# colmap/glomap

Hardware: NVIDIA H100
Metric: observations/sec per BA LM-iteration (higher is better)
Workload: dtype f64

## Files before the change

glomap_b200/csrc/ba_kernels.cuh:

```cuda
#pragma once
#include "common.cuh"
#include "pcg.cuh"

namespace b200 {

constexpr int kCamRec = 8;
constexpr int kIntrRec = 8;
constexpr double kZEps = 1e-12;
constexpr int kSeg = 256;
__host__ __device__ constexpr int seg_split(int n) { return n <= 0 ? 0 : (n < kSeg + kSeg / 2 ? 1 : (n + kSeg / 2) / kSeg); }
constexpr int kIntrSmem = 16;
constexpr int kJpDoubles = 6;
constexpr int kSensorRec = 16;

struct BAView {
  int C, P, K;
  long long N;
  int n_tiles;
  int n_segs;
  int min_views;
  const int* obs_cam;
  const int* obs_pt;
  const double2* obs_xy;
  const unsigned* pt_begin;
// ... 35 lines not shown
  }
}

struct Intr {
  double fx, fy, cx, cy, k1, k2;
  int model;
};
__device__ __forceinline__ Intr ld_intr(const double* __restrict__ ir) {
  return Intr{ir[0], ir[1], ir[2], ir[3], ir[4], ir[5], (int)ir[6]};
}

struct ProjJac {
  double iz, u, v, m00, m01, m10, m11;
};

__device__ __forceinline__ void project_jac(const Intr& in, double x, double y, double z, double& px, double& py,
                                            ProjJac& pj) {
  const double iz = 1.0 / z;
  const double u = x * iz, v = y * iz;
  pj.iz = iz;
  pj.u = u;
  pj.v = v;
  if (in.k1 == 0.0 && in.k2 == 0.0) {
    px = in.fx * u + in.cx;
    py = in.fy * v + in.cy;
    pj.m00 = in.fx; pj.m01 = 0.0; pj.m10 = 0.0; pj.m11 = in.fy;
  } else {
    const double r2 = u * u + v * v;
    const double d = 1.0 + r2 * (in.k1 + in.k2 * r2);
    const double dd = in.k1 + 2.0 * in.k2 * r2;
    px = in.fx * u * d + in.cx;
    py = in.fy * v * d + in.cy;
    const double a00 = d + 2.0 * u * u * dd, a01 = 2.0 * u * v * dd, a11 = d + 2.0 * v * v * dd;
    pj.m00 = in.fx * a00; pj.m01 = in.fx * a01; pj.m10 = in.fy * a01; pj.m11 = in.fy * a11;
  }
}
__device__ __forceinline__ void project_only(const Intr& in, double x, double y, double z, double& px, double& py) {
  const double iz = 1.0 / z;
  const double u = x * iz, v = y * iz;
  if (in.k1 == 0.0 && in.k2 == 0.0) {
    px = in.fx * u + in.cx;
    py = in.fy * v + in.cy;
  } else {
    const double r2 = u * u + v * v;
    const double d = 1.0 + r2 * (in.k1 + in.k2 * r2);
    px = in.fx * u * d + in.cx;
    py = in.fy * v * d + in.cy;
  }
}
// ... 91 lines not shown
  for (int a = 0; a < 2; ++a) {
    const double j0 = J[3 * a], j1 = J[3 * a + 1], j2 = J[3 * a + 2];
    o.Jr[3 * a + 0] = rvar ? -2.0 * (j1 * rz - j2 * ry) : 0.0;
    o.Jr[3 * a + 1] = rvar ? -2.0 * (j2 * rx - j0 * rz) : 0.0;
    o.Jr[3 * a + 2] = rvar ? -2.0 * (j0 * ry - j1 * rx) : 0.0;
  }
#pragma unroll
  for (int a = 0; a < 2; ++a)
#pragma unroll
    for (int b = 0; b < 3; ++b) o.Jp[3 * a + b] = J[3 * a] * R[b] + J[3 * a + 1] * R[3 + b] + J[3 * a + 2] * R[6 + b];
}

struct ObsCore {
  double J[6], e[2], rho0, rho1, RX[3], R[9];
  double uv[2];
  ProjJac pj;
  bool valid;
};
__device__ __forceinline__ void obs_core_R(const double R[9], const double4& t4, const Intr& in,
                                           const double* __restrict__ sr, double X0, double X1, double X2, double2 xy,
                                           double huber_a, ObsCore& o) {
#pragma unroll
  for (int k = 0; k < 9; ++k) o.R[k] = R[k];
  o.RX[0] = o.R[0] * X0 + o.R[1] * X1 + o.R[2] * X2;
  o.RX[1] = o.R[3] * X0 + o.R[4] * X1 + o.R[5] * X2;
  o.RX[2] = o.R[6] * X0 + o.R[7] * X1 + o.R[8] * X2;
  double xc = o.RX[0] + t4.x, yc = o.RX[1] + t4.y, zc = o.RX[2] + t4.z;
  if (sr) sensor_apply(sr, xc, yc, zc);
  o.valid = zc > kZEps;
  if (!o.valid) {
#pragma unroll
    for (int k = 0; k < 6; ++k) o.J[k] = 0.0;
    o.e[0] = o.e[1] = 0.0;
    o.rho0 = 0.0;
    o.rho1 = 0.0;
    o.uv[0] = o.uv[1] = 0.0;
    o.pj = ProjJac{0.0, 0.0, 0.0, 0.0, 0.0, 0.0, 0.0};
    return;
  }
  double px, py;
  project_jac(in, xc, yc, zc, px, py, o.pj);
  proj_jac_rows(o.pj, o.J);
  o.uv[0] = xc / zc;
  o.uv[1] = yc / zc;
  if (sr) {
#pragma unroll
    for (int a = 0; a < 2; ++a) {
      const double j0 = o.J[3 * a], j1 = o.J[3 * a + 1], j2 = o.J[3 * a + 2];
      o.J[3 * a] = j0 * sr[0] + j1 * sr[3] + j2 * sr[6];
      o.J[3 * a + 1] = j0 * sr[1] + j1 * sr[4] + j2 * sr[7];
      o.J[3 * a + 2] = j0 * sr[2] + j1 * sr[5] + j2 * sr[8];
    }
  }
  o.e[0] = px - xy.x;
// ... 755 lines not shown
```

glomap_b200/csrc/ba_kernels_v2.cuh:

```cuda
#pragma once
#include "ba_kernels.cuh"
#include "pcg.cuh"

namespace b200 {

struct BAViewV2 {
  const double* Ap;
  double* z4;
  const double* pts4;
  double* Ufk = nullptr;
  const IntrVarRec* ivar = nullptr;
  int C = 0;
};

template <int NK>
__device__ __forceinline__ void obs_intr_jac(const ObsCore& o, const Intr& in, const IntrVarRec& iv,
                                             double Jk[2][NK > 0 ? NK : 1]) {
#pragma unroll
  for (int j = 0; j < NK; ++j) {
    double jx = 0.0, jy = 0.0;
    if (j < iv.mb) intr_param_jac(in, iv.pidx[j], o.uv[0], o.uv[1], 1.0, jx, jy);
    if (!o.valid) jx = jy = 0.0;
    Jk[0][j] = jx;
    Jk[1][j] = jy;
  }
}
template <int NK>
__device__ __forceinline__ void obs_intr_rows(const ObsCore& o, const Intr& in, const IntrVarRec& iv,
                                              const double Jp[6], double Jk[2][NK > 0 ? NK : 1],
                                              double B[NK > 0 ? 3 * NK : 1]) {
  obs_intr_jac<NK>(o, in, iv, Jk);
#pragma unroll
  for (int j = 0; j < NK; ++j)
#pragma unroll
    for (int c = 0; c < 3; ++c) B[3 * j + c] = o.rho1 * (Jp[c] * Jk[0][j] + Jp[3 + c] * Jk[1][j]);
}

struct SegRec {
  double R[9];
  double4 t4;
  Intr in;
  const double* sr;
};
__device__ __forceinline__ void seg_records(const BAView& v, int seg, int cam, const double* __restrict__ cam_rec,
                                            const double* __restrict__ intr_rec, SegRec& s) {
  const double4 q4 = ld_rec32(cam_rec + (size_t)cam * kCamRec);
  s.t4 = ld_rec32(cam_rec + (size_t)cam * kCamRec + 4);
  s.in = ld_intr(intr_rec + (size_t)v.seg_intr[seg] * kIntrRec);
  s.sr = sensor_of_seg(v, seg);
  const double q[4] = {q4.x, q4.y, q4.z, q4.w};
  quat_to_R(q, s.R);
}
__device__ __forceinline__ void to_sensor(const double* __restrict__ sr, double x[3]) {
  if (!sr) return;
  const double x0 = x[0], x1 = x[1], x2 = x[2];
#pragma unroll
  for (int k = 0; k < 3; ++k) x[k] = sr[3 * k] * x0 + sr[3 * k + 1] * x1 + sr[3 * k + 2] * x2;
}
__device__ __forceinline__ void cam_frame_jac(const ObsCore& o, const double r[3], double a[2], double w[3]) {
  const ProjJac& p = o.pj;
  const double t0 = r[0] - p.u * r[2], t1 = r[1] - p.v * r[2];
  const double c = o.rho1 * p.iz;
  a[0] = c * (p.m00 * t0 + p.m01 * t1);
  a[1] = c * (p.m10 * t0 + p.m11 * t1);
  const double s0 = p.iz * (p.m00 * a[0] + p.m10 * a[1]), s1 = p.iz * (p.m01 * a[0] + p.m11 * a[1]);
  w[0] = s0;
  w[1] = s1;
  w[2] = -(p.u * s0 + p.v * s1);
}
__device__ __forceinline__ void rig_to_frame(const double* __restrict__ sr, double x[3]) {
  const double x0 = x[0], x1 = x[1], x2 = x[2];
#pragma unroll
  for (int k = 0; k < 3; ++k) x[k] = sr[k] * x0 + sr[3 + k] * x1 + sr[6 + k] * x2;
}

constexpr int kXqStride = 8;
__global__ void ba2_pack_x(int C, const double* __restrict__ x, const double* __restrict__ cam_rec,
                           double* __restrict__ xp) {
  const int c = blockIdx.x * blockDim.x + threadIdx.x;
  if (c >= C) return;
  const double* r = cam_rec + (size_t)c * kCamRec;
  const double q[4] = {r[0], r[1], r[2], r[3]};
  double R[9];
// ... 68 lines not shown
  const bool tvar = !(cmask & 2), rvar = !(cmask & 1);
  constexpr int NKK = NK > 0 ? NK : 1;
  const int blk = v.seg_intr[warp];
  IntrVarRec iv{};
  if (NK > 0) iv = v2.ivar[blk];
  double Ukk[NKK * (NKK + 1) / 2], gk[NKK], Ufk[6][NKK];
#pragma unroll
  for (int k = 0; k < NKK * (NKK + 1) / 2; ++k) Ukk[k] = 0.0;
#pragma unroll
  for (int k = 0; k < NKK; ++k) {
    gk[k] = 0.0;
#pragma unroll
    for (int i2 = 0; i2 < 6; ++i2) Ufk[i2][k] = 0.0;
  }
  const double* __restrict__ pts4 = v2.pts4;
  int i = b + lane;
  int pt_nxt = 0;
  double2 xy = make_double2(0, 0);
  double4 Xc = make_double4(0, 0, 0, 0);
  if (i < e) {
    const int pt0 = ld_stream(v.pt_c + i);
    if (i + 32 < e) pt_nxt = ld_stream(v.pt_c + i + 32);
    xy = ld_stream(v.xy_c + i);
    Xc = ld_rec32(pts4 + 4 * (size_t)pt0);
  }
  for (; i < e; i += 32) {
    double4 Xn = Xc;
    double2 xyn = xy;
    int pt_nn = 0;
    if (i + 32 < e) {
      Xn = ld_rec32(pts4 + 4 * (size_t)pt_nxt);
      xyn = ld_stream(v.xy_c + i + 32);
    }
    if (i + 64 < e) pt_nn = ld_stream(v.pt_c + i + 64);
    const double X0 = Xc.x, X1 = Xc.y, X2 = Xc.z;
    ObsCore o;
    obs_core_R(sg.R, sg.t4, sg.in, sg.sr, X0, X1, X2, xy, huber_a, o);
    double Jc[2][6];
#pragma unroll
    for (int a = 0; a < 2; ++a) {
      const double j0 = o.J[3 * a], j1 = o.J[3 * a + 1], j2 = o.J[3 * a + 2];
      Jc[a][0] = rvar ? -2.0 * (j1 * o.RX[2] - j2 * o.RX[1]) : 0.0;
      Jc[a][1] = rvar ? -2.0 * (j2 * o.RX[0] - j0 * o.RX[2]) : 0.0;
      Jc[a][2] = rvar ? -2.0 * (j0 * o.RX[1] - j1 * o.RX[0]) : 0.0;
      Jc[a][3] = tvar ? j0 : 0.0;
      Jc[a][4] = tvar ? j1 : 0.0;
      Jc[a][5] = tvar ? j2 : 0.0;
    }
    const double e0 = o.rho1 * o.e[0], e1 = o.rho1 * o.e[1];
    int idx = 0;
#pragma unroll
    for (int i2 = 0; i2 < 6; ++i2) {
// ... 38 lines not shown
    }
  }
#pragma unroll
  for (int k = 0; k < 21; ++k) {
    const double s = warp_sum(U[k]);
    if (lane == k && s != 0.0) atomicAdd(&v.U[(size_t)cam * 21 + k], s);
  }
#pragma unroll
  for (int k = 0; k < 6; ++k) {
    const double s = warp_sum(g[k]);
    if (lane == 21 + k && s != 0.0) atomicAdd(&v.gc[(size_t)cam * 6 + k], s);
  }
}

__global__ void __launch_bounds__(128, B200_SD_MIN_CTAS) ba2_schur_diag(BAView v, BAViewV2 v2, const double* __restrict__ cam_rec,
                                                                        const double* __restrict__ intr_rec, double huber_a) {
  const int warp = (blockIdx.x * blockDim.x + threadIdx.x) >> 5;
  const int lane = threadIdx.x & 31;
  if (warp >= v.n_segs) return;
  const int cam = v.seg_cam[warp];
  const int b = v.seg_begin[warp], e = v.seg_end[warp];
  SegRec sg;
  seg_records(v, warp, cam, cam_rec, intr_rec, sg);
  double RR[6] = {0, 0, 0, 0, 0, 0}, RT[9] = {0, 0, 0, 0, 0, 0, 0, 0, 0}, TT[6] = {0, 0, 0, 0, 0, 0};
  int i = b + lane;
  int pt_nxt = 0;
  double2 xy = make_double2(0, 0), va = xy, vb = xy, vc = xy;
  double4 Xc = make_double4(0, 0, 0, 0);
  if (i < e) {
    const int pt0 = ld_stream(v.pt_c + i);
    if (i + 32 < e) pt_nxt = ld_stream(v.pt_c + i + 32);
    xy = ld_stream(v.xy_c + i);
    Xc = ld_rec32(v2.pts4 + 4 * (size_t)pt0);
    const double2* vp = reinterpret_cast<const double2*>(v.Vinv + (size_t)pt0 * 6);
    va = vp[0]; vb = vp[1]; vc = vp[2];
  }
  for (; i < e; i += 32) {
    double4 Xn = Xc;
    double2 xyn = xy, van = va, vbn = vb, vcn = vc;
    int pt_nn = 0;
    if (i + 32 < e) {
      Xn = ld_rec32(v2.pts4 + 4 * (size_t)pt_nxt);
      xyn = ld_stream(v.xy_c + i + 32);
      const double2* vp = reinterpret_cast<const double2*>(v.Vinv + (size_t)pt_nxt * 6);
      van = vp[0]; vbn = vp[1]; vcn = vp[2];
    }
    if (i + 64 < e) pt_nn = ld_stream(v.pt_c + i + 64);
    ObsCore o;
    obs_core_R(sg.R, sg.t4, sg.in, sg.sr, Xc.x, Xc.y, Xc.z, xy, huber_a, o);
    double X[3] = {o.RX[0], o.RX[1], o.RX[2]};
    to_sensor(sg.sr, X);
    const ProjJac& pj = o.pj;
    const double vi[6] = {va.x, va.y, vb.x, vb.y, vc.x, vc.y};
    double e0[3] = {1.0, 0.0, -pj.u}, e1[3] = {0.0, 1.0, -pj.v};
    if (sg.sr) {
#pragma unroll
      for (int c = 0; c < 3; ++c) {
        e0[c] = sg.sr[c] - pj.u * sg.sr[6 + c];
        e1[c] = sg.sr[3 + c] - pj.v * sg.sr[6 + c];
      }
    }
    double l0[3], l1[3], t0[3], t1[3];
#pragma unroll
    for (int c = 0; c < 3; ++c) {
      l0[c] = e0[0] * sg.R[c] + e0[1] * sg.R[3 + c] + e0[2] * sg.R[6 + c];
      l1[c] = e1[0] * sg.R[c] + e1[1] * sg.R[3 + c] + e1[2] * sg.R[6 + c];
    }
    sym3_mul(vi, l0, t0);
    sym3_mul(vi, l1, t1);
    const double q00 = l0[0] * t0[0] + l0[1] * t0[1] + l0[2] * t0[2];
    const double q01 = l0[0] * t1[0] + l0[1] * t1[1] + l0[2] * t1[2];
    const double q11 = l1[0] * t1[0] + l1[1] * t1[1] + l1[2] * t1[2];
    const double k00 = pj.m00 * pj.m00 + pj.m10 * pj.m10, k01 = pj.m00 * pj.m01 + pj.m10 * pj.m11,
                 k11 = pj.m01 * pj.m01 + pj.m11 * pj.m11;
    const double a00 = k00 * q00 + k01 * q01, a01 = k00 * q01 + k01 * q11;
    const double a10 = k01 * q00 + k11 * q01, a11 = k01 * q01 + k11 * q11;
    const double sc = o.rho1 * pj.iz * pj.iz, c2 = sc * sc;
    const double h00 = c2 * (a00 * k00 + a01 * k01), h01 = c2 * (a00 * k01 + a01 * k11), h11 = c2 * (a10 * k01 + a11 * k11);
    double N[3][3];
    N[0][0] = h00; N[0][1] = N[1][0] = h01; N[1][1] = h11;
    N[0][2] = N[2][0] = -(h00 * pj.u + h01 * pj.v);
    N[1][2] = N[2][1] = -(h01 * pj.u + h11 * pj.v);
    N[2][2] = -(N[0][2] * pj.u + N[1][2] * pj.v);
    double P[3][3];
#pragma unroll
    for (int c = 0; c < 3; ++c) {
      const double n0 = N[0][c], n1 = N[1][c], n2 = N[2][c];
      P[0][c] = 2.0 * (X[1] * n2 - X[2] * n1);
      P[1][c] = 2.0 * (X[2] * n0 - X[0] * n2);
      P[2][c] = 2.0 * (X[0] * n1 - X[1] * n0);
    }
    double PK[3][3];
#pragma unroll
    for (int r = 0; r < 3; ++r) {
      PK[r][0] = P[r][1] * X[2] - P[r][2] * X[1];
      PK[r][1] = -P[r][0] * X[2] + P[r][2] * X[0];
      PK[r][2] = P[r][0] * X[1] - P[r][1] * X[0];
    }
    RR[0] += -2.0 * PK[0][0]; RR[1] += -2.0 * PK[0][1]; RR[2] += -2.0 * PK[0][2];
    RR[3] += -2.0 * PK[1][1]; RR[4] += -2.0 * PK[1][2]; RR[5] += -2.0 * PK[2][2];
#pragma unroll
    for (int r = 0; r < 3; ++r)
#pragma unroll
      for (int c = 0; c < 3; ++c) RT[3 * r + c] += P[r][c];
    TT[0] += N[0][0]; TT[1] += N[0][1]; TT[2] += N[0][2]; TT[3] += N[1][1]; TT[4] += N[1][2]; TT[5] += N[2][2];
    Xc = Xn; xy = xyn; va = van; vb = vbn; vc = vcn; pt_nxt = pt_nn;
  }
#pragma unroll
  for (int k = 0; k < 6; ++k) RR[k] = warp_sum(RR[k]);
#pragma unroll
  for (int k = 0; k < 9; ++k) RT[k] = warp_sum(RT[k]);
#pragma unroll
  for (int k = 0; k < 6; ++k) TT[k] = warp_sum(TT[k]);
  if (lane == 0) {
    const int mask = (int)(__double_as_longlong(sg.t4.w) & 0xff);
    double R[9] = {1, 0, 0, 0, 1, 0, 0, 0, 1};
    if (sg.sr) {
      for (int r = 0; r < 3; ++r)
        for (int c = 0; c < 3; ++c) R[3 * r + c] = sg.sr[3 * c + r];
    }
    double M[6][6];
// ... 199 lines not shown
__global__ void ba2_point_rhs_z(BAView v, BAViewV2 v2) {
  const int p = blockIdx.x * blockDim.x + threadIdx.x;
  if (p >= v.P) return;
  double vi[6], g[3], z[3];
#pragma unroll
  for (int k = 0; k < 6; ++k) vi[k] = v.Vinv[6 * (size_t)p + k];
#pragma unroll
  for (int k = 0; k < 3; ++k) g[k] = v.gp[3 * (size_t)p + k];
  sym3_mul(vi, g, z);
  const bool pvalid = (int)(v.pt_begin[p + 1] - v.pt_begin[p]) >= v.min_views;
  *reinterpret_cast<double4*>(v2.z4 + 4 * (size_t)p) = pvalid ? make_double4(z[0], z[1], z[2], 0.0) : make_double4(0, 0, 0, 0);
}

template <int NK>
__global__ void __launch_bounds__(128, B200_PB_MIN_CTAS) ba2_pass_b(BAView v, BAViewV2 v2, const double* __restrict__ cam_rec,
                                                 const double* __restrict__ intr_rec, double huber_a,
                                                 double* __restrict__ y, const PcgCtl* __restrict__ ctl, int seg_lo,
                                                 int seg_hi) {
  if (ctl && ctl->done) return;
  const int warp = seg_lo + ((blockIdx.x * blockDim.x + threadIdx.x) >> 5);
  const int lane = threadIdx.x & 31;
  if (warp >= seg_hi) return;
  const int cam = v.seg_cam[warp];
  const int b = v.seg_begin[warp], e = v.seg_end[warp];
  const int blk = v.seg_intr[warp];
  SegRec sg;
  seg_records(v, warp, cam, cam_rec, intr_rec, sg);
  constexpr int NKK = NK > 0 ? NK : 1;
  IntrVarRec iv{};
  if (NK > 0) iv = v2.ivar[blk];
  double acc[6] = {0, 0, 0, 0, 0, 0};
  double accK[NKK];
#pragma unroll
  for (int k = 0; k < NKK; ++k) accK[k] = 0.0;
  const uint64_t keep = l2_policy_evict_last();
  int i = b + lane;
  int pt_nxt = 0;
  double4 X = make_double4(0, 0, 0, 0), z = X;
  double2 xy = make_double2(0, 0);
  if (i < e) {
    const int pt0 = ld_stream(v.pt_c + i);
    if (i + 32 < e) pt_nxt = ld_stream(v.pt_c + i + 32);
    X = ld_rec32(v2.pts4 + 4 * (size_t)pt0);
    z = ld_keep4(v2.z4 + 4 * (size_t)pt0, keep);
    xy = ld_stream(v.xy_c + i);
  }
  for (; i < e; i += 32) {
    double4 Xn = X, zn = z;
    double2 xyn = xy;
    int pt_nn = 0;
    if (i + 32 < e) {
      Xn = ld_rec32(v2.pts4 + 4 * (size_t)pt_nxt);
      zn = ld_keep4(v2.z4 + 4 * (size_t)pt_nxt, keep);
      xyn = ld_stream(v.xy_c + i + 32);
    }
    if (i + 64 < e) pt_nn = ld_stream(v.pt_c + i + 64);
    ObsCore o;
    obs_core_R(sg.R, sg.t4, sg.in, sg.sr, X.x, X.y, X.z, xy, huber_a, o);
    double P[3] = {o.RX[0], o.RX[1], o.RX[2]};
    to_sensor(sg.sr, P);
    double r[3] = {sg.R[0] * z.x + sg.R[1] * z.y + sg.R[2] * z.z,
                   sg.R[3] * z.x + sg.R[4] * z.y + sg.R[5] * z.z,
                   sg.R[6] * z.x + sg.R[7] * z.y + sg.R[8] * z.z};
    to_sensor(sg.sr, r);
    double a[2], w[3];
    cam_frame_jac(o, r, a, w);
    acc[0] += P[1] * w[2] - P[2] * w[1];
    acc[1] += P[2] * w[0] - P[0] * w[2];
    acc[2] += P[0] * w[1] - P[1] * w[0];
    acc[3] += w[0];
    acc[4] += w[1];
    acc[5] += w[2];
    if (NK > 0) {
      double Jk[2][NKK];
      obs_intr_jac<NK>(o, sg.in, iv, Jk);
#pragma unroll
      for (int k = 0; k < NK; ++k) accK[k] += Jk[0][k] * a[0] + Jk[1][k] * a[1];
    }
    X = Xn; z = zn; xy = xyn; pt_nxt = pt_nn;
  }
#pragma unroll
  for (int k = 0; k < 6; ++k) acc[k] = warp_sum(acc[k]);
  if (sg.sr) {
    rig_to_frame(sg.sr, acc);
    rig_to_frame(sg.sr, acc + 3);
  }
  const int mask = (int)(__double_as_longlong(sg.t4.w) & 0xff);
#pragma unroll
  for (int k = 0; k < 6; ++k) {
    const double s = k < 3 ? 2.0 * acc[k] : acc[k];
    const bool fixed = k < 3 ? (mask & 1) : (mask & 2);
    if (lane == k && !fixed && s != 0.0) atomicAdd(&y[(size_t)cam * 6 + k], -s);
  }
  if (NK > 0) {
// ... 70 lines not shown
```

glomap_b200/csrc/ba_solver.cuh:

```cuda
#pragma once
#include <cub/cub.cuh>

#include <algorithm>
#include <climits>
#include <cmath>
#include <cstdlib>
#include <vector>

#include "../../include/b200sfm_testing.h"
#include "ba_kernels.cuh"
#include "ba_kernels_v2.cuh"
#include "ba_kernels_v3.cuh"
#include "ba_kernels_ext.cuh"
#include "filter_kernels.cuh"
#include "processor_kernels.cuh"
#include "context.cuh"
#include "pcg.cuh"

namespace b200 {

constexpr double kSliceL2Share = 1.0 / 6.0;

__global__ void k_expand_obs_pt(int P, const unsigned* __restrict__ pt_begin, int* __restrict__ obs_pt) {
  const int p = blockIdx.x * blockDim.x + threadIdx.x;
// ... 129 lines not shown
  bool use_v2 = false;
  bool use_ell = false;
  int ell_groups = 0, ell_ctas = 0, ell_bpart_rows = 0;
  long long ell_rows = 0;
  DevBuf<int> ell_row0, ell_pt, ell_len, ell_slot, ell_cam;
  DevBuf<double2> ell_xy;
  DevBuf<unsigned short> ell_sensor;
  DevBuf<double> ell_A, ell_part;
  b200::EllView ell_view() {
    b200::EllView e;
    e.n_groups = ell_groups; e.row0 = ell_row0.p; e.pt = ell_pt.p; e.len = ell_len.p; e.cam = ell_cam.p; e.xy = ell_xy.p;
    e.sensor = S > 0 ? ell_sensor.p : nullptr; e.A = ell_A.p; e.B = kfast ? ell_B.p : nullptr;
    return e;
  }
  DevBuf<double> z4, pts4, xq, bpart, bpart2;
  size_t smem_k3v2 = 0;
  bool kfast = false;
  int nk = 0;
  DevBuf<double> ell_B, Ufk;
  b200::BAViewV2 view2() {
    b200::BAViewV2 w;
    w.Ap = W.p; w.z4 = z4.p; w.pts4 = pts4.p;
    w.Ufk = kfast ? Ufk.p : nullptr; w.ivar = ivar.p; w.C = C;
    return w;
  }
  int cur = 0;
  DevBuf<double> cam_rec, intr_rec;
  DevBuf<double> W, V, Vinv, gp, lin , Sd, Minv, jscale_c, jscale_p, Dc;
  DevBuf<double> px, pr, pz, pp, pq, yw, bvec;
  DevBuf<double> scal;
  b200::EventTimer timer_lin, timer_mv;
  size_t smem_k1 = 0, smem_k3 = 0;

  double* U() { return lin.p; }
  double* gc() { return lin.p + (size_t)CB * 21; }
  double* cost_ptr() { return lin.p + (size_t)CB * 27; }

// ... 513 lines not shown
      else if (ext_s) B200_EXT_A(false, true);
      else B200_EXT_A(false, false);
#undef B200_EXT_A
    }
    if (n_segs > 0) {
#define B200_EXT_B(WK, WS)                                                                                              \
  B200_LAUNCH(ctx, (bax_pass_b<WK, WS>), sgrid, 128, 0, v, ex, view2(), cam_rec.p, intr_rec.p, points[cur].p, x, huber_a, y, ctl)
      if (ext_k && ext_s) B200_EXT_B(true, true);
      else if (ext_k) B200_EXT_B(true, false);
      else if (ext_s) B200_EXT_B(false, true);
      else B200_EXT_B(false, false);
#undef B200_EXT_B
    }
  }

  void launch_pass_b(const b200::BAView& v, double huber_a, double* y, const b200::PcgCtl* ctl, int seg_lo = 0,
                     int seg_hi = -1) {
    using namespace b200;
    if (seg_hi < 0) seg_hi = n_segs;
    if (seg_hi <= seg_lo) return;
    const int grid = cdiv((long long)(seg_hi - seg_lo) * 32, 128);
#define B200_PASS_B(NKV) \
  B200_LAUNCH(ctx, ba2_pass_b<NKV>, grid, 128, 0, v, view2(), cam_rec.p, intr_rec.p, huber_a, y, ctl, seg_lo, seg_hi)
    if (kfast && nk == 2) B200_PASS_B(2);
    else if (kfast) B200_PASS_B(1);
    else B200_PASS_B(0);
#undef B200_PASS_B
  }
  void launch_pass_a0(const b200::BAView& v, double radius, const b200::PcgCtl* ctl) {
    using namespace b200;
    if (kfast && nk == 2)
      B200_LAUNCH(ctx, (ba3_pass_a<0, 2>), ell_ctas, kEllThreads, 0, v, ell_view(), view2(), xq.p, points[cur].p, nullptr, radius, nullptr, ctl);
    else if (kfast)
      B200_LAUNCH(ctx, (ba3_pass_a<0, 1>), ell_ctas, kEllThreads, 0, v, ell_view(), view2(), xq.p, points[cur].p, nullptr, radius, nullptr, ctl);
    else
      B200_LAUNCH(ctx, (ba3_pass_a<0, 0>), ell_ctas, kEllThreads, 0, v, ell_view(), view2(), xq.p, points[cur].p, nullptr, radius, nullptr, ctl);
  }
  void launch_cross(const double* x, double* y, const b200::PcgCtl* ctl) {
// ... 18 lines not shown
      e0 = timer_mv.next();
      e1 = timer_mv.next();
      B200_CUDA_OK(cudaEventRecord(e0, s));
    }
    if (matrix_free()) {
      ext_matvec(x, y, o.thres_loss_function, radius, points_var, ctl);
    } else if (kfast && !points_var) {
      launch_cross(x, y, ctl);
    } else if (use_v2) {
      if (use_ell)
        launch_pass_a0(v, radius, ctl);
      else
        B200_LAUNCH(ctx, ba2_pass_a<0>, n_tiles, kTile, smem_k3v2, v, view2(), xq.p, points[cur].p, nullptr, radius, nullptr, ctl);
      if (kfast) launch_cross(x, y, ctl);
      if (split_ar) {
        launch_pass_b(v, o.thres_loss_function, y, ctl, 0, seg_mid);
        B200_CUDA_OK(cudaEventRecord(ctx->ev_half, s));
        B200_CUDA_OK(cudaStreamWaitEvent(ctx->comm_stream, ctx->ev_half, 0));
        ctx->allreduce_sum_on(ctx->comm_stream, y, (size_t)(C / 2) * 6);
        B200_CUDA_OK(cudaEventRecord(ctx->ev_comm, ctx->comm_stream));
        launch_pass_b(v, o.thres_loss_function, y, ctl, seg_mid, n_segs);
      } else if (n_segs > 0) {
        launch_pass_b(v, o.thres_loss_function, y, ctl);
      }
    } else {
      B200_LAUNCH(ctx, ba_schur_pass<0>, n_tiles, kTile, smem_k3, v, x, y, nullptr, nullptr, radius, nullptr, nullptr,
                  nullptr, 0, ctl);
    }
    if (profile) B200_CUDA_OK(cudaEventRecord(e1, s));
    if (split_ar) {
      ctx->allreduce_sum(y + (size_t)(C / 2) * 6, nB6 - (size_t)(C / 2) * 6);
      B200_CUDA_OK(cudaStreamWaitEvent(s, ctx->ev_comm, 0));
    } else {
      ctx->allreduce_sum(y, nB6);
    }
  }

  StepResult compute_step(const b200sfm_ba_opts& o, double radius, bool points_var, bool set_jscale_p, bool profile) {
    using namespace b200;
    cudaStream_t s = ctx->stream;
    BAView v = view();
    const int nB6 = nbk * 6;
    if (points_var) B200_LAUNCH(ctx, ba_damp_points, cdiv(P, 256), 256, 0, P, V.p, jscale_p.p, set_jscale_p ? 1 : 0, radius, Vinv.p);
    B200_LAUNCH(ctx, ba_damp_cams, cdiv(nB6, 256), 256, 0, nbk, U(), jscale_c.p, radius, Dc.p);
    const bool recomp = matrix_free();
    const bool schur_jacobi = schur_jacobi_on(o, points_var);
    double* yrhs = Sd.p + (size_t)CB * 21;
    Sd.zero(s);
    if (schur_jacobi && n_segs > 0) {
      if (use_v2)
        B200_LAUNCH(ctx, ba2_schur_diag, cdiv((long long)n_segs * 32, 128), 128, 0, v, view2(), cam_rec.p, intr_rec.p,
                    o.thres_loss_function);
      else B200_LAUNCH(ctx, ba_schur_diag, cdiv((long long)n_segs * 32, 128), 128, 0, v);
    }
    if (points_var) {
      if (use_v2) {
        B200_LAUNCH(ctx, ba2_point_rhs_z, cdiv(P, 256), 256, 0, v, view2());
        if (recomp) ext_matvec(nullptr, yrhs, o.thres_loss_function, radius, true, nullptr);
        else if (n_segs > 0) launch_pass_b(v, o.thres_loss_function, yrhs, nullptr);
      } else {
        B200_LAUNCH(ctx, ba_schur_pass<1>, n_tiles, kTile, smem_k3, v, nullptr, yrhs, nullptr, nullptr, radius, nullptr);
      }
    } else if (recomp) {
      z4.zero(s);
    }
    if (schur_jacobi || points_var) ctx->allreduce_sum(Sd.p, (size_t)CB * 27);
    B200_LAUNCH(ctx, ba_build_precond, cdiv(nbk, 128), 128, 0, nbk, U(), Dc.p, schur_jacobi ? Sd.p : nullptr, Minv.p);
    B200_LAUNCH(ctx, k_rhs, cdiv(nB6, 256), 256, 0, nB6, gc(), points_var ? yrhs : nullptr, bvec.p);
    const int max_it = std::max(1, o.pcg_max_iterations);
    const int nblk = cdiv(nbk, kPcgThreads);
    ctx->pcgh.ensure(max_it, (size_t)nblk * 3, ctx->world);
    double* part_pq = ctx->pcgh.d_part;
    double* part_rz = ctx->pcgh.d_part + nblk;
    double* part_rr = ctx->pcgh.d_part + 2 * (size_t)nblk;
// ... 126 lines not shown
      for (int i = 0; i < S; ++i) ext_s = ext_s || h_sensor_var[i] != 0;
    ext = ext_k || ext_s;
    nbk = ext ? CB : C;
    B200_CUDA_OK(cudaStreamSynchronize(s));
    use_v2 = ext || (o.design != 1);
    use_ell = use_v2 && (ext || !(getenv("B200SFM_ELL") && atoi(getenv("B200SFM_ELL")) == 0));
    nk = 0;
    if (ext_k)
      for (int k = 0; k < K; ++k) nk = std::max(nk, h_ivar[k].mb);
    kfast = ext_k && !ext_s && S == 0 && nk <= 2 && !(getenv("B200SFM_KFAST") && atoi(getenv("B200SFM_KFAST")) == 0);
    if (kfast) {
      const size_t cells = (size_t)std::max<long long>(ell_rows, 1) * 32;
      if (ell_B.n < cells * 3 * nk) ell_B.alloc(cells * 3 * nk);
      if (Ufk.n < (size_t)C * 6 * nk) Ufk.alloc((size_t)C * 6 * nk);
    }
  }
  void launch_eff_mask(const b200sfm_ba_opts& o) {
    B200_LAUNCH(ctx, b200::k_eff_mask, b200::cdiv(C, 256), 256, 0, C, cam_mask_base.p, o.optimize_rotations ? 0 : 1,
                o.optimize_translation ? 0 : 1, cam_mask.p);
  }

  void reject_step() { build_records(cur); }

  int solve(const b200sfm_ba_opts& o, b200sfm_lm_stats* st) {
    using namespace b200;
    cudaStream_t s = ctx->stream;
    select_paths(o);
    const bool l2_persist = use_v2 && !(getenv("B200SFM_L2_PERSIST") && atoi(getenv("B200SFM_L2_PERSIST")) == 0) &&
                            l2_persist_window(s, ctx->device, z4.p, z4.bytes());
    const long long launches0 = ctx->launches;
// ... 162 lines not shown
```

Baseline: 1.552 billion.

## Cache per-observation projection data for reuse in Schur diag and pass-B kernels

```diff
diff --git a/glomap_b200/csrc/ba_kernels.cuh b/glomap_b200/csrc/ba_kernels.cuh
--- a/glomap_b200/csrc/ba_kernels.cuh
+++ b/glomap_b200/csrc/ba_kernels.cuh
@@ -73,6 +73,16 @@
   double iz, u, v, m00, m01, m10, m11;
 };
 
+__device__ __forceinline__ double radial_m(const Intr& in, double u, double v, double& m00, double& m01, double& m10,
+                                           double& m11) {
+  const double r2 = u * u + v * v;
+  const double d = 1.0 + r2 * (in.k1 + in.k2 * r2);
+  const double dd = in.k1 + 2.0 * in.k2 * r2;
+  const double a00 = d + 2.0 * u * u * dd, a01 = 2.0 * u * v * dd, a11 = d + 2.0 * v * v * dd;
+  m00 = in.fx * a00; m01 = in.fx * a01; m10 = in.fy * a01; m11 = in.fy * a11;
+  return d;
+}
+
 __device__ __forceinline__ void project_jac(const Intr& in, double x, double y, double z, double& px, double& py,
                                             ProjJac& pj) {
   const double iz = 1.0 / z;
@@ -85,13 +95,9 @@
     py = in.fy * v + in.cy;
     pj.m00 = in.fx; pj.m01 = 0.0; pj.m10 = 0.0; pj.m11 = in.fy;
   } else {
-    const double r2 = u * u + v * v;
-    const double d = 1.0 + r2 * (in.k1 + in.k2 * r2);
-    const double dd = in.k1 + 2.0 * in.k2 * r2;
+    const double d = radial_m(in, u, v, pj.m00, pj.m01, pj.m10, pj.m11);
     px = in.fx * u * d + in.cx;
     py = in.fy * v * d + in.cy;
-    const double a00 = d + 2.0 * u * u * dd, a01 = 2.0 * u * v * dd, a11 = d + 2.0 * v * v * dd;
-    pj.m00 = in.fx * a00; pj.m01 = in.fx * a01; pj.m10 = in.fy * a01; pj.m11 = in.fy * a11;
   }
 }
 __device__ __forceinline__ void project_only(const Intr& in, double x, double y, double z, double& px, double& py) {
@@ -213,6 +219,7 @@
 struct ObsCore {
   double J[6], e[2], rho0, rho1, RX[3], R[9];
   double uv[2];
+  double zc;
   ProjJac pj;
   bool valid;
 };
@@ -234,9 +241,11 @@
     o.rho0 = 0.0;
     o.rho1 = 0.0;
     o.uv[0] = o.uv[1] = 0.0;
+    o.zc = 0.0;
     o.pj = ProjJac{0.0, 0.0, 0.0, 0.0, 0.0, 0.0, 0.0};
     return;
   }
+  o.zc = zc;
   double px, py;
   project_jac(in, xc, yc, zc, px, py, o.pj);
   proj_jac_rows(o.pj, o.J);
diff --git a/glomap_b200/csrc/ba_kernels_v2.cuh b/glomap_b200/csrc/ba_kernels_v2.cuh
--- a/glomap_b200/csrc/ba_kernels_v2.cuh
+++ b/glomap_b200/csrc/ba_kernels_v2.cuh
@@ -8,22 +8,31 @@
   const double* Ap;
   double* z4;
   const double* pts4;
+  double* prj = nullptr;
+  int Nv = 0;
   double* Ufk = nullptr;
   const IntrVarRec* ivar = nullptr;
   int C = 0;
 };
 
 template <int NK>
+__device__ __forceinline__ void intr_jac_uv(double u, double v, const Intr& in, const IntrVarRec& iv,
+                                            double Jk[2][NK > 0 ? NK : 1]) {
+#pragma unroll
+  for (int j = 0; j < NK; ++j) {
+    double jx = 0.0, jy = 0.0;
+    if (j < iv.mb) intr_param_jac(in, iv.pidx[j], u, v, 1.0, jx, jy);
+    Jk[0][j] = jx;
+    Jk[1][j] = jy;
+  }
+}
+template <int NK>
 __device__ __forceinline__ void obs_intr_jac(const ObsCore& o, const Intr& in, const IntrVarRec& iv,
                                              double Jk[2][NK > 0 ? NK : 1]) {
-#pragma unroll
-  for (int j = 0; j < NK; ++j) {
-    double jx = 0.0, jy = 0.0;
-    if (j < iv.mb) intr_param_jac(in, iv.pidx[j], o.uv[0], o.uv[1], 1.0, jx, jy);
-    if (!o.valid) jx = jy = 0.0;
-    Jk[0][j] = jx;
-    Jk[1][j] = jy;
-  }
+  intr_jac_uv<NK>(o.uv[0], o.uv[1], in, iv, Jk);
+#pragma unroll
+  for (int j = 0; j < NK; ++j)
+    if (!o.valid) Jk[0][j] = Jk[1][j] = 0.0;
 }
 template <int NK>
 __device__ __forceinline__ void obs_intr_rows(const ObsCore& o, const Intr& in, const IntrVarRec& iv,
@@ -51,22 +60,55 @@
   const double q[4] = {q4.x, q4.y, q4.z, q4.w};
   quat_to_R(q, s.R);
 }
-__device__ __forceinline__ void to_sensor(const double* __restrict__ sr, double x[3]) {
-  if (!sr) return;
-  const double x0 = x[0], x1 = x[1], x2 = x[2];
-#pragma unroll
-  for (int k = 0; k < 3; ++k) x[k] = sr[3 * k] * x0 + sr[3 * k + 1] * x1 + sr[3 * k + 2] * x2;
-}
-__device__ __forceinline__ void cam_frame_jac(const ObsCore& o, const double r[3], double a[2], double w[3]) {
-  const ProjJac& p = o.pj;
-  const double t0 = r[0] - p.u * r[2], t1 = r[1] - p.v * r[2];
-  const double c = o.rho1 * p.iz;
-  a[0] = c * (p.m00 * t0 + p.m01 * t1);
-  a[1] = c * (p.m10 * t0 + p.m11 * t1);
-  const double s0 = p.iz * (p.m00 * a[0] + p.m10 * a[1]), s1 = p.iz * (p.m01 * a[0] + p.m11 * a[1]);
+__device__ __forceinline__ void seg_sensor_frame(const SegRec& s, double Rs[9], double tp[3]) {
+  const double t[3] = {s.t4.x, s.t4.y, s.t4.z};
+#pragma unroll
+  for (int k = 0; k < 9; ++k) Rs[k] = s.R[k];
+#pragma unroll
+  for (int k = 0; k < 3; ++k) tp[k] = t[k];
+  if (!s.sr) return;
+  const double* __restrict__ sr = s.sr;
+#pragma unroll
+  for (int r = 0; r < 3; ++r) {
+#pragma unroll
+    for (int c = 0; c < 3; ++c) Rs[3 * r + c] = sr[3 * r] * s.R[c] + sr[3 * r + 1] * s.R[3 + c] + sr[3 * r + 2] * s.R[6 + c];
+    tp[r] = sr[3 * r] * t[0] + sr[3 * r + 1] * t[1] + sr[3 * r + 2] * t[2] + sr[9 + r];
+  }
+}
+struct PrjRec {
+  double u, v, zc, c;
+};
+__device__ __forceinline__ PrjRec ld_prj(const double* __restrict__ prj, size_t nv, int i) {
+  return PrjRec{ld_stream(prj + i), ld_stream(prj + nv + i), ld_stream(prj + 2 * nv + i), ld_stream(prj + 3 * nv + i)};
+}
+__device__ __forceinline__ void prj_m(const PrjRec& q, const Intr& in, bool radial, double& m00, double& m01,
+                                      double& m10, double& m11) {
+  m00 = in.fx; m01 = 0.0; m10 = 0.0; m11 = in.fy;
+  if (radial) radial_m(in, q.u, q.v, m00, m01, m10, m11);
+}
+template <bool RADIAL>
+__device__ __forceinline__ void prj_jac(const PrjRec& q, const Intr& in, const double r[3], double a[2], double w[3]) {
+  const double t0 = r[0] - q.u * r[2], t1 = r[1] - q.v * r[2];
+  double mt0, mt1, s0, s1;
+  if (RADIAL) {
+    double m00, m01, m10, m11;
+    prj_m(q, in, true, m00, m01, m10, m11);
+    mt0 = m00 * t0 + m01 * t1;
+    mt1 = m10 * t0 + m11 * t1;
+    s0 = q.c * (m00 * mt0 + m10 * mt1);
+    s1 = q.c * (m01 * mt0 + m11 * mt1);
+  } else {
+    mt0 = in.fx * t0;
+    mt1 = in.fy * t1;
+    s0 = q.c * (in.fx * mt0);
+    s1 = q.c * (in.fy * mt1);
+  }
   w[0] = s0;
   w[1] = s1;
-  w[2] = -(p.u * s0 + p.v * s1);
+  w[2] = -(q.u * s0 + q.v * s1);
+  const double cz = q.c * q.zc;
+  a[0] = cz * mt0;
+  a[1] = cz * mt1;
 }
 __device__ __forceinline__ void rig_to_frame(const double* __restrict__ sr, double x[3]) {
   const double x0 = x[0], x1 = x[1], x2 = x[2];
@@ -165,6 +207,8 @@
     for (int i2 = 0; i2 < 6; ++i2) Ufk[i2][k] = 0.0;
   }
   const double* __restrict__ pts4 = v2.pts4;
+  double* __restrict__ prj = v2.prj;
+  const size_t nv = (size_t)v2.Nv;
   int i = b + lane;
   int pt_nxt = 0;
   double2 xy = make_double2(0, 0);
@@ -187,6 +231,10 @@
     const double X0 = Xc.x, X1 = Xc.y, X2 = Xc.z;
     ObsCore o;
     obs_core_R(sg.R, sg.t4, sg.in, sg.sr, X0, X1, X2, xy, huber_a, o);
+    st_stream(prj + i, o.pj.u);
+    st_stream(prj + nv + i, o.pj.v);
+    st_stream(prj + 2 * nv + i, o.zc);
+    st_stream(prj + 3 * nv + i, o.rho1 * o.pj.iz * o.pj.iz);
     double Jc[2][6];
 #pragma unroll
     for (int a = 0; a < 2; ++a) {
@@ -255,7 +303,7 @@
 }
 
 __global__ void __launch_bounds__(128, B200_SD_MIN_CTAS) ba2_schur_diag(BAView v, BAViewV2 v2, const double* __restrict__ cam_rec,
-                                                                        const double* __restrict__ intr_rec, double huber_a) {
+                                                                        const double* __restrict__ intr_rec) {
   const int warp = (blockIdx.x * blockDim.x + threadIdx.x) >> 5;
   const int lane = threadIdx.x & 31;
   if (warp >= v.n_segs) return;
@@ -263,66 +311,58 @@
   const int b = v.seg_begin[warp], e = v.seg_end[warp];
   SegRec sg;
   seg_records(v, warp, cam, cam_rec, intr_rec, sg);
+  double Rs[9], tp[3];
+  seg_sensor_frame(sg, Rs, tp);
+  const bool radial = !(sg.in.k1 == 0.0 && sg.in.k2 == 0.0);
   double RR[6] = {0, 0, 0, 0, 0, 0}, RT[9] = {0, 0, 0, 0, 0, 0, 0, 0, 0}, TT[6] = {0, 0, 0, 0, 0, 0};
+  const double* __restrict__ prj = v2.prj;
+  const size_t nv = (size_t)v2.Nv;
   int i = b + lane;
   int pt_nxt = 0;
-  double2 xy = make_double2(0, 0), va = xy, vb = xy, vc = xy;
-  double4 Xc = make_double4(0, 0, 0, 0);
+  double2 va = make_double2(0, 0), vb = va, vc = va;
+  PrjRec q{0.0, 0.0, 0.0, 0.0};
   if (i < e) {
     const int pt0 = ld_stream(v.pt_c + i);
     if (i + 32 < e) pt_nxt = ld_stream(v.pt_c + i + 32);
-    xy = ld_stream(v.xy_c + i);
-    Xc = ld_rec32(v2.pts4 + 4 * (size_t)pt0);
+    q = ld_prj(prj, nv, i);
     const double2* vp = reinterpret_cast<const double2*>(v.Vinv + (size_t)pt0 * 6);
     va = vp[0]; vb = vp[1]; vc = vp[2];
   }
   for (; i < e; i += 32) {
-    double4 Xn = Xc;
-    double2 xyn = xy, van = va, vbn = vb, vcn = vc;
+    PrjRec qn = q;
+    double2 van = va, vbn = vb, vcn = vc;
     int pt_nn = 0;
     if (i + 32 < e) {
-      Xn = ld_rec32(v2.pts4 + 4 * (size_t)pt_nxt);
-      xyn = ld_stream(v.xy_c + i + 32);
+      qn = ld_prj(prj, nv, i + 32);
       const double2* vp = reinterpret_cast<const double2*>(v.Vinv + (size_t)pt_nxt * 6);
       van = vp[0]; vbn = vp[1]; vcn = vp[2];
     }
     if (i + 64 < e) pt_nn = ld_stream(v.pt_c + i + 64);
-    ObsCore o;
-    obs_core_R(sg.R, sg.t4, sg.in, sg.sr, Xc.x, Xc.y, Xc.z, xy, huber_a, o);
-    double X[3] = {o.RX[0], o.RX[1], o.RX[2]};
-    to_sensor(sg.sr, X);
-    const ProjJac& pj = o.pj;
+    const double X[3] = {q.zc * q.u - tp[0], q.zc * q.v - tp[1], q.zc - tp[2]};
+    double m00, m01, m10, m11;
+    prj_m(q, sg.in, radial, m00, m01, m10, m11);
     const double vi[6] = {va.x, va.y, vb.x, vb.y, vc.x, vc.y};
-    double e0[3] = {1.0, 0.0, -pj.u}, e1[3] = {0.0, 1.0, -pj.v};
-    if (sg.sr) {
-#pragma unroll
-      for (int c = 0; c < 3; ++c) {
-        e0[c] = sg.sr[c] - pj.u * sg.sr[6 + c];
-        e1[c] = sg.sr[3 + c] - pj.v * sg.sr[6 + c];
-      }
-    }
     double l0[3], l1[3], t0[3], t1[3];
 #pragma unroll
     for (int c = 0; c < 3; ++c) {
-      l0[c] = e0[0] * sg.R[c] + e0[1] * sg.R[3 + c] + e0[2] * sg.R[6 + c];
-      l1[c] = e1[0] * sg.R[c] + e1[1] * sg.R[3 + c] + e1[2] * sg.R[6 + c];
+      l0[c] = Rs[c] - q.u * Rs[6 + c];
+      l1[c] = Rs[3 + c] - q.v * Rs[6 + c];
     }
     sym3_mul(vi, l0, t0);
     sym3_mul(vi, l1, t1);
     const double q00 = l0[0] * t0[0] + l0[1] * t0[1] + l0[2] * t0[2];
     const double q01 = l0[0] * t1[0] + l0[1] * t1[1] + l0[2] * t1[2];
     const double q11 = l1[0] * t1[0] + l1[1] * t1[1] + l1[2] * t1[2];
-    const double k00 = pj.m00 * pj.m00 + pj.m10 * pj.m10, k01 = pj.m00 * pj.m01 + pj.m10 * pj.m11,
-                 k11 = pj.m01 * pj.m01 + pj.m11 * pj.m11;
+    const double k00 = m00 * m00 + m10 * m10, k01 = m00 * m01 + m10 * m11, k11 = m01 * m01 + m11 * m11;
     const double a00 = k00 * q00 + k01 * q01, a01 = k00 * q01 + k01 * q11;
     const double a10 = k01 * q00 + k11 * q01, a11 = k01 * q01 + k11 * q11;
-    const double sc = o.rho1 * pj.iz * pj.iz, c2 = sc * sc;
+    const double c2 = q.c * q.c;
     const double h00 = c2 * (a00 * k00 + a01 * k01), h01 = c2 * (a00 * k01 + a01 * k11), h11 = c2 * (a10 * k01 + a11 * k11);
     double N[3][3];
     N[0][0] = h00; N[0][1] = N[1][0] = h01; N[1][1] = h11;
-    N[0][2] = N[2][0] = -(h00 * pj.u + h01 * pj.v);
-    N[1][2] = N[2][1] = -(h01 * pj.u + h11 * pj.v);
-    N[2][2] = -(N[0][2] * pj.u + N[1][2] * pj.v);
+    N[0][2] = N[2][0] = -(h00 * q.u + h01 * q.v);
+    N[1][2] = N[2][1] = -(h01 * q.u + h11 * q.v);
+    N[2][2] = -(N[0][2] * q.u + N[1][2] * q.v);
     double P[3][3];
 #pragma unroll
     for (int c = 0; c < 3; ++c) {
@@ -345,7 +385,7 @@
 #pragma unroll
       for (int c = 0; c < 3; ++c) RT[3 * r + c] += P[r][c];
     TT[0] += N[0][0]; TT[1] += N[0][1]; TT[2] += N[0][2]; TT[3] += N[1][1]; TT[4] += N[1][2]; TT[5] += N[2][2];
-    Xc = Xn; xy = xyn; va = van; vb = vbn; vc = vcn; pt_nxt = pt_nn;
+    q = qn; va = van; vb = vbn; vc = vcn; pt_nxt = pt_nn;
   }
 #pragma unroll
   for (int k = 0; k < 6; ++k) RR[k] = warp_sum(RR[k]);
@@ -575,9 +615,8 @@
 
 template <int NK>
 __global__ void __launch_bounds__(128, B200_PB_MIN_CTAS) ba2_pass_b(BAView v, BAViewV2 v2, const double* __restrict__ cam_rec,
-                                                 const double* __restrict__ intr_rec, double huber_a,
-                                                 double* __restrict__ y, const PcgCtl* __restrict__ ctl, int seg_lo,
-                                                 int seg_hi) {
+                                                 const double* __restrict__ intr_rec, double* __restrict__ y,
+                                                 const PcgCtl* __restrict__ ctl, int seg_lo, int seg_hi) {
   if (ctl && ctl->done) return;
   const int warp = seg_lo + ((blockIdx.x * blockDim.x + threadIdx.x) >> 5);
   const int lane = threadIdx.x & 31;
@@ -587,6 +626,9 @@
   const int blk = v.seg_intr[warp];
   SegRec sg;
   seg_records(v, warp, cam, cam_rec, intr_rec, sg);
+  double Rs[9], tp[3];
+  seg_sensor_frame(sg, Rs, tp);
+  const bool radial = !(sg.in.k1 == 0.0 && sg.in.k2 == 0.0);
   constexpr int NKK = NK > 0 ? NK : 1;
   IntrVarRec iv{};
   if (NK > 0) iv = v2.ivar[blk];
@@ -595,37 +637,37 @@
 #pragma unroll
   for (int k = 0; k < NKK; ++k) accK[k] = 0.0;
   const uint64_t keep = l2_policy_evict_last();
+  const double* __restrict__ prj = v2.prj;
+  const size_t nv = (size_t)v2.Nv;
   int i = b + lane;
   int pt_nxt = 0;
-  double4 X = make_double4(0, 0, 0, 0), z = X;
-  double2 xy = make_double2(0, 0);
+  double4 z = make_double4(0, 0, 0, 0);
+  PrjRec q{0.0, 0.0, 0.0, 0.0}, qn = q;
   if (i < e) {
     const int pt0 = ld_stream(v.pt_c + i);
-    if (i + 32 < e) pt_nxt = ld_stream(v.pt_c + i + 32);
-    X = ld_rec32(v2.pts4 + 4 * (size_t)pt0);
+    if (i + 32 < e) {
+      pt_nxt = ld_stream(v.pt_c + i + 32);
+      qn = ld_prj(prj, nv, i + 32);
+    }
     z = ld_keep4(v2.z4 + 4 * (size_t)pt0, keep);
-    xy = ld_stream(v.xy_c + i);
+    q = ld_prj(prj, nv, i);
   }
   for (; i < e; i += 32) {
-    double4 Xn = X, zn = z;
-    double2 xyn = xy;
+    double4 zn = z;
+    PrjRec qnn = qn;
     int pt_nn = 0;
-    if (i + 32 < e) {
-      Xn = ld_rec32(v2.pts4 + 4 * (size_t)pt_nxt);
-      zn = ld_keep4(v2.z4 + 4 * (size_t)pt_nxt, keep);
-      xyn = ld_stream(v.xy_c + i + 32);
-    }
-    if (i + 64 < e) pt_nn = ld_stream(v.pt_c + i + 64);
-    ObsCore o;
-    obs_core_R(sg.R, sg.t4, sg.in, sg.sr, X.x, X.y, X.z, xy, huber_a, o);
-    double P[3] = {o.RX[0], o.RX[1], o.RX[2]};
-    to_sensor(sg.sr, P);
-    double r[3] = {sg.R[0] * z.x + sg.R[1] * z.y + sg.R[2] * z.z,
-                   sg.R[3] * z.x + sg.R[4] * z.y + sg.R[5] * z.z,
-                   sg.R[6] * z.x + sg.R[7] * z.y + sg.R[8] * z.z};
-    to_sensor(sg.sr, r);
+    if (i + 32 < e) zn = ld_keep4(v2.z4 + 4 * (size_t)pt_nxt, keep);
+    if (i + 64 < e) {
+      pt_nn = ld_stream(v.pt_c + i + 64);
+      qnn = ld_prj(prj, nv, i + 64);
+    }
+    const double r[3] = {Rs[0] * z.x + Rs[1] * z.y + Rs[2] * z.z,
+                         Rs[3] * z.x + Rs[4] * z.y + Rs[5] * z.z,
+                         Rs[6] * z.x + Rs[7] * z.y + Rs[8] * z.z};
     double a[2], w[3];
-    cam_frame_jac(o, r, a, w);
+    if (radial) prj_jac<true>(q, sg.in, r, a, w);
+    else prj_jac<false>(q, sg.in, r, a, w);
+    const double P[3] = {q.zc * q.u - tp[0], q.zc * q.v - tp[1], q.zc - tp[2]};
     acc[0] += P[1] * w[2] - P[2] * w[1];
     acc[1] += P[2] * w[0] - P[0] * w[2];
     acc[2] += P[0] * w[1] - P[1] * w[0];
@@ -634,11 +676,11 @@
     acc[5] += w[2];
     if (NK > 0) {
       double Jk[2][NKK];
-      obs_intr_jac<NK>(o, sg.in, iv, Jk);
+      intr_jac_uv<NK>(q.u, q.v, sg.in, iv, Jk);
 #pragma unroll
       for (int k = 0; k < NK; ++k) accK[k] += Jk[0][k] * a[0] + Jk[1][k] * a[1];
     }
-    X = Xn; z = zn; xy = xyn; pt_nxt = pt_nn;
+    z = zn; q = qn; qn = qnn; pt_nxt = pt_nn;
   }
 #pragma unroll
   for (int k = 0; k < 6; ++k) acc[k] = warp_sum(acc[k]);
diff --git a/glomap_b200/csrc/ba_solver.cuh b/glomap_b200/csrc/ba_solver.cuh
--- a/glomap_b200/csrc/ba_solver.cuh
+++ b/glomap_b200/csrc/ba_solver.cuh
@@ -167,13 +167,14 @@
     return e;
   }
   DevBuf<double> z4, pts4, xq, bpart, bpart2;
+  DevBuf<double> prj;
   size_t smem_k3v2 = 0;
   bool kfast = false;
   int nk = 0;
   DevBuf<double> ell_B, Ufk;
   b200::BAViewV2 view2() {
     b200::BAViewV2 w;
-    w.Ap = W.p; w.z4 = z4.p; w.pts4 = pts4.p;
+    w.Ap = W.p; w.z4 = z4.p; w.pts4 = pts4.p; w.prj = prj.p; w.Nv = Nv;
     w.Ufk = kfast ? Ufk.p : nullptr; w.ivar = ivar.p; w.C = C;
     return w;
   }
@@ -717,14 +718,13 @@
     }
   }
 
-  void launch_pass_b(const b200::BAView& v, double huber_a, double* y, const b200::PcgCtl* ctl, int seg_lo = 0,
-                     int seg_hi = -1) {
+  void launch_pass_b(const b200::BAView& v, double* y, const b200::PcgCtl* ctl, int seg_lo = 0, int seg_hi = -1) {
     using namespace b200;
     if (seg_hi < 0) seg_hi = n_segs;
     if (seg_hi <= seg_lo) return;
     const int grid = cdiv((long long)(seg_hi - seg_lo) * 32, 128);
 #define B200_PASS_B(NKV) \
-  B200_LAUNCH(ctx, ba2_pass_b<NKV>, grid, 128, 0, v, view2(), cam_rec.p, intr_rec.p, huber_a, y, ctl, seg_lo, seg_hi)
+  B200_LAUNCH(ctx, ba2_pass_b<NKV>, grid, 128, 0, v, view2(), cam_rec.p, intr_rec.p, y, ctl, seg_lo, seg_hi)
     if (kfast && nk == 2) B200_PASS_B(2);
     else if (kfast) B200_PASS_B(1);
     else B200_PASS_B(0);
@@ -773,14 +773,14 @@
         B200_LAUNCH(ctx, ba2_pass_a<0>, n_tiles, kTile, smem_k3v2, v, view2(), xq.p, points[cur].p, nullptr, radius, nullptr, ctl);
       if (kfast) launch_cross(x, y, ctl);
       if (split_ar) {
-        launch_pass_b(v, o.thres_loss_function, y, ctl, 0, seg_mid);
+        launch_pass_b(v, y, ctl, 0, seg_mid);
         B200_CUDA_OK(cudaEventRecord(ctx->ev_half, s));
         B200_CUDA_OK(cudaStreamWaitEvent(ctx->comm_stream, ctx->ev_half, 0));
         ctx->allreduce_sum_on(ctx->comm_stream, y, (size_t)(C / 2) * 6);
         B200_CUDA_OK(cudaEventRecord(ctx->ev_comm, ctx->comm_stream));
-        launch_pass_b(v, o.thres_loss_function, y, ctl, seg_mid, n_segs);
+        launch_pass_b(v, y, ctl, seg_mid, n_segs);
       } else if (n_segs > 0) {
-        launch_pass_b(v, o.thres_loss_function, y, ctl);
+        launch_pass_b(v, y, ctl);
       }
     } else {
       B200_LAUNCH(ctx, ba_schur_pass<0>, n_tiles, kTile, smem_k3, v, x, y, nullptr, nullptr, radius, nullptr, nullptr,
@@ -808,15 +808,14 @@
     Sd.zero(s);
     if (schur_jacobi && n_segs > 0) {
       if (use_v2)
-        B200_LAUNCH(ctx, ba2_schur_diag, cdiv((long long)n_segs * 32, 128), 128, 0, v, view2(), cam_rec.p, intr_rec.p,
-                    o.thres_loss_function);
+        B200_LAUNCH(ctx, ba2_schur_diag, cdiv((long long)n_segs * 32, 128), 128, 0, v, view2(), cam_rec.p, intr_rec.p);
       else B200_LAUNCH(ctx, ba_schur_diag, cdiv((long long)n_segs * 32, 128), 128, 0, v);
     }
     if (points_var) {
       if (use_v2) {
         B200_LAUNCH(ctx, ba2_point_rhs_z, cdiv(P, 256), 256, 0, v, view2());
         if (recomp) ext_matvec(nullptr, yrhs, o.thres_loss_function, radius, true, nullptr);
-        else if (n_segs > 0) launch_pass_b(v, o.thres_loss_function, yrhs, nullptr);
+        else if (n_segs > 0) launch_pass_b(v, yrhs, nullptr);
       } else {
         B200_LAUNCH(ctx, ba_schur_pass<1>, n_tiles, kTile, smem_k3, v, nullptr, yrhs, nullptr, nullptr, radius, nullptr);
       }
@@ -973,6 +972,7 @@
       if (ell_B.n < cells * 3 * nk) ell_B.alloc(cells * 3 * nk);
       if (Ufk.n < (size_t)C * 6 * nk) Ufk.alloc((size_t)C * 6 * nk);
     }
+    if (use_v2 && !matrix_free() && prj.n < (size_t)std::max(Nv, 1) * 4) prj.alloc((size_t)std::max(Nv, 1) * 4);
   }
   void launch_eff_mask(const b200sfm_ba_opts& o) {
     B200_LAUNCH(ctx, b200::k_eff_mask, b200::cdiv(C, 256), 256, 0, C, cam_mask_base.p, o.optimize_rotations ? 0 : 1,
diff --git a/profiles/ab_bench.py b/profiles/ab_bench.py
--- /dev/null
+++ b/profiles/ab_bench.py
@@ -0,0 +1,89 @@
+#!/usr/bin/env python
+import argparse
+import json
+import os
+import statistics
+import subprocess
+import sys
+import tempfile
+
+import numpy as np
+
+CASES = [("config4", []), ("config4_intr", ["--optimize-intrinsics", "1"]), ("config2", ["--workload", "config2"])]
+BENCH = ["--gpus", "1", "--steps", "3", "--warmup", "3", "--no-cpu-baseline"]
+
+
+def run(cmd, cwd):
+    r = subprocess.run(cmd, cwd=cwd, capture_output=True, text=True)
+    if r.returncode != 0:
+        raise SystemExit(f"{' '.join(cmd)} in {cwd} failed ({r.returncode}):\n{r.stdout[-3000:]}\n{r.stderr[-3000:]}")
+    return r.stdout
+
+
+def bench_line(tree, args, dump=None):
+    cmd = [sys.executable, "bench.py"] + BENCH + args + (["--dump-outputs", dump] if dump else [])
+    out = run(cmd, tree)
+    return json.loads([ln for ln in out.splitlines() if ln.startswith("{")][-1])
+
+
+def max_rel_diff(da, db):
+    res = {}
+    for f in sorted(os.listdir(da)):
+        if not f.endswith(".npy") or not os.path.exists(os.path.join(db, f)):
+            continue
+        a, b = np.load(os.path.join(da, f)), np.load(os.path.join(db, f))
+        res[f[:-4]] = float(np.abs(a - b).max() / max(np.abs(a).max(), 1e-300)) if a.size else 0.0
+    return res
+
+
+def main():
+    ap = argparse.ArgumentParser()
+    ap.add_argument("--base", required=True)
+    ap.add_argument("--change", required=True)
+    ap.add_argument("--rounds", type=int, default=3)
+    ap.add_argument("--out", default=None)
+    a = ap.parse_args()
+    trees = {"base": os.path.abspath(a.base), "change": os.path.abspath(a.change)}
+
+    if a.out:
+        os.makedirs(a.out, exist_ok=True)
+
+    def say(s=""):
+        print(s, flush=True)
+        if a.out:
+            with open(os.path.join(a.out, "ab_bench.txt"), "a") as f:
+                f.write(s + "\n")
+
+    say(run(["nvidia-smi", "--query-gpu=name,power.limit,clocks.max.sm", "--format=csv"], ".").strip())
+    ms = {(c, t): [] for c, _ in CASES for t in trees}
+    its, parity = {}, {}
+    with tempfile.TemporaryDirectory() as tmp:
+        for r in range(a.rounds):
+            for t, tree in trees.items():
+                for c, extra in CASES:
+                    dump = os.path.join(tmp, f"{t}{r}_{c}") if r < 2 else None
+                    ln = bench_line(tree, extra, dump)
+                    ms[(c, t)].append(ln["ms_per_step"])
+                    cfg = ln["config"]
+                    its[(c, t)] = (cfg["lm_iterations_per_step"], cfg["lm_iterations_per_step"] * cfg["pcg_iterations_per_lm_iteration"])
+                    parity[(c, t)] = ln.get("parity", {}).get("checked")
+                    say(f"round {r} {t:6s} {c:13s} ms_per_step {ln['ms_per_step']:.3f}  LM/PCG per step {its[(c, t)]}")
+        say("\n| case | base ms_per_step (runs) | change ms_per_step (runs) | median change | LM/PCG base | LM/PCG change | parity checked base/change |")
+        say("|---|---|---|---|---|---|---|")
+        for c, _ in CASES:
+            b, ch = ms[(c, "base")], ms[(c, "change")]
+            mb, mc = statistics.median(b), statistics.median(ch)
+            say(f"| {c} | {mb:.2f} ({', '.join(f'{x:.2f}' for x in b)}) | {mc:.2f} ({', '.join(f'{x:.2f}' for x in ch)}) | "
+                f"{100 * (mc / mb - 1):+.1f} % | {its[(c, 'base')]} | {its[(c, 'change')]} | "
+                f"{parity[(c, 'base')]}/{parity[(c, 'change')]} |")
+        say("\nmax |x - y| / max |y| of the dumped results: change vs base (round 0), and base round 1 vs base round 0")
+        for c, _ in CASES:
+            say(f"{c}: change {max_rel_diff(os.path.join(tmp, f'change0_{c}'), os.path.join(tmp, f'base0_{c}'))}")
+            say(f"{c}: base   {max_rel_diff(os.path.join(tmp, f'base1_{c}'), os.path.join(tmp, f'base0_{c}'))}")
+    for t, tree in trees.items():
+        say(f"\n## kernel_times.py, {t}")
+        say(run([sys.executable, "profiles/kernel_times.py", "--workload", "config4", "--top", "16"], tree))
+
+
+if __name__ == "__main__":
+    main()
```

After: 1.594 billion, median of 6. 2.7% higher.
